# Zhijian-Mei/py-debruijn

Hardware: AMD Instinct MI355X
Metric: k-mers/s hashed+graph-built at k=31 (higher is better)
Workload: dtype u64; 1 GPU; 10000000 x 150 bp synthetic reads (10000000 per GPU): BASELINE.json configs[1]; k=31, 30x coverage of a 50000000 bp uniform genome, 1% substitutions, seed 1; k=31, reads_per_gpu=10000000, reads_total=10000000, read_len=150, parallelism=single table

## Files before the change

py-debruijn_amd/_dbg.py:

```python
from __future__ import annotations

import ctypes as C
import os

import numpy as np

_HERE = os.path.dirname(os.path.abspath(__file__))
LIB_PATH = os.environ.get("DBG_LIB") or os.path.join(_HERE, "libdbg_hip.so")

DBG_OK, DBG_E_ARG, DBG_E_HIP, DBG_E_ALPHABET, DBG_E_CAPACITY, DBG_E_NOMEM = 0, -1, -2, -3, -4, -5
F_INDEG, F_KEEP_MASK, F_KEEP_SHIFT, F_BRANCH, F_PULLED = 0x01, 0x1E, 1, 0x20, 0x40
NO_NODE = 0xFFFFFFFF
ABI_VERSION = 6

SYMBOLS = (
    "dbg_create", "dbg_destroy", "dbg_last_error", "dbg_abi_version", "dbg_set_option", "dbg_set_reads", "dbg_set_reads_fasta",
    "dbg_set_reads_fasta_file", "dbg_fasta_ingest_stats", "dbg_set_reads_fastq_file", "dbg_fastq_ingest_stats",
    "dbg_set_reads_fasta_records", "dbg_set_reads_fasta_records_file", "dbg_fasta_records_stats", "dbg_write_contigs_fasta_wrapped",
    "dbg_set_reads_device",
    "dbg_synth_reads", "dbg_reads_checksum", "dbg_copy_reads", "dbg_reads_device", "dbg_build", "dbg_refine_edge_order", "dbg_export_orders",
    "dbg_get_alphabet", "dbg_export_keepmask", "dbg_export_dict_order",
    "dbg_prune", "dbg_remove_tips",
    "dbg_mark_pull_reads", "dbg_walk", "dbg_get_sizes", "dbg_get_stats", "dbg_get_counter", "dbg_export_nodes", "dbg_export_keys_hi",
    "dbg_export_succ",
# ... 71 lines not shown
    _fields_ = [(n, C.c_uint64) for n in (
        "bytes_written", "chunks", "chunk_bytes", "peak_device_bytes", "lift_bytes")] + [
        (n, C.c_double) for n in ("ms_total", "ms_io_wait", "ms_fill", "ms_d2h")]

    def as_dict(self):
        return {n: getattr(self, n) for n, _ in self._fields_}


class SplitStats(C.Structure):
    _fields_ = [(n, C.c_uint64) for n in (
        "n_reads_in", "n_bytes_in", "n_reads_out", "n_bytes_out", "n_cut_bytes", "n_folded_bytes", "n_reads_changed",
        "n_reads_emptied", "changed", "peak_extra_device_bytes")]

    def as_dict(self):
        return {n: getattr(self, n) for n, _ in self._fields_}


SPLIT_FOLD_CASE = 1
SPLIT_WORD_BYTES = 64
SPLIT_BLOCK_BYTES = 256 * 4 * SPLIT_WORD_BYTES
SPLIT_ROUND_BYTES = 256 * SPLIT_BLOCK_BYTES


class RevcompStats(C.Structure):
    _fields_ = [(n, C.c_uint64) for n in (
        "n_reads_in", "n_bytes_in", "n_reads_out", "n_bytes_out", "n_other_bytes", "n_palindromes",
        "peak_extra_device_bytes")] + [("ms_kernel", C.c_double)]

    def as_dict(self):
        return {n: getattr(self, n) for n, _ in self._fields_}


RC_TILE_BYTES = 256 * 8 * 16
RC_SLICE_READS = 1024


class Spectrum(C.Structure):
    _fields_ = [(n, C.c_uint64) for n in ("n_nodes", "n_edges", "sum_edge_counts", "max_edge_count", "max_out_weight")] + [
        ("D", C.c_uint64 * 33), ("K", C.c_uint64 * 33)] + [
        (n, C.c_uint64) for n in ("pruned", "n_bins", "peak_extra_device_bytes")] + [("ms_kernel", C.c_double)]

    def as_dict(self):
        return {n: (np.array(getattr(self, n), dtype=np.uint64) if n in ("D", "K") else getattr(self, n)) for n, _ in self._fields_}


SP_LDS_BINS = 1024
SP_MAX_BINS = 1 << 20


class WalkBlock(C.Structure):
    _fields_ = [("src", C.c_void_p), ("contigs", C.c_void_p), ("n", C.c_uint64)]


COUNTERS = ("extract_presplit_fallbacks", "extract_presplit_rehists", "resolve_direct_hits", "resolve_keyed",
            "refine_crowded", "pull_crowded", "lookup_index_builds", "lookup_dir_calls", "lookup_index_calls",
            "part_lookup_calls", "count_events", "count_extra_ranges", "count_retries_query_cap", "count_retries_node_cap",
            "count_retries_counter16")


class DbgError(RuntimeError):
    def __init__(self, code, msg):
        super().__init__(f"dbg error {code}: {msg}")
        self.code = code


class AlphabetError(DbgError, ValueError):
    pass


_lib = None


def load_library():
    global _lib
    if _lib is not None:
        return _lib
    if not os.path.exists(LIB_PATH):
        raise OSError(f"{LIB_PATH} not found: build it with py-debruijn_amd/csrc/build.sh "
                      f"(there is no CPU fallback for the device path)")
    try:
        import torch
    except ImportError:
        pass
    lib = C.CDLL(LIB_PATH)
    H = C.c_void_p
    u64p, u32p, u8p = C.POINTER(C.c_uint64), C.POINTER(C.c_uint32), C.POINTER(C.c_uint8)
    vp = C.c_void_p
    sig = {
        "dbg_create": (C.c_int, [C.c_int, C.POINTER(H)]),
        "dbg_destroy": (None, [H]),
        "dbg_last_error": (C.c_char_p, [H]),
        "dbg_abi_version": (C.c_int, []),
        "dbg_set_option": (C.c_int, [H, C.c_char_p, C.c_int64]),
        "dbg_set_reads": (C.c_int, [H, vp, vp, C.c_uint64]),
        "dbg_set_reads_fasta": (C.c_int, [H, vp, C.c_uint64]),
        "dbg_set_reads_fasta_file": (C.c_int, [H, C.c_char_p, C.c_uint64, C.c_uint64, C.c_uint64]),
        "dbg_fasta_ingest_stats": (C.c_int, [H, C.POINTER(IngestStats)]),
        "dbg_set_reads_fastq_file": (C.c_int, [H, C.c_char_p, C.c_uint64, C.c_uint64, C.c_uint64, C.c_uint32]),
        "dbg_fastq_ingest_stats": (C.c_int, [H, C.POINTER(FastqStats)]),
        "dbg_set_reads_fasta_records": (C.c_int, [H, vp, C.c_uint64]),
        "dbg_set_reads_fasta_records_file": (C.c_int, [H, C.c_char_p, C.c_uint64, C.c_uint64, C.c_uint64]),
        "dbg_fasta_records_stats": (C.c_int, [H, C.POINTER(FastaRecordsStats)]),
        "dbg_set_reads_device": (C.c_int, [H, vp, C.c_uint64, vp, C.c_uint64]),
        "dbg_synth_reads": (C.c_int, [H, C.c_uint64, C.c_uint64, C.c_uint64, C.c_uint64, C.c_uint32, C.c_uint32]),
        "dbg_reads_checksum": (C.c_int, [H, u64p]),
        "dbg_copy_reads": (C.c_int, [H, vp, vp]),
        "dbg_build": (C.c_int, [H, C.c_int, C.c_uint64]),
# ... 965 lines not shown
```

py-debruijn_amd/csrc/dbg_hip.hip:

```cpp
#include <hip/hip_runtime.h>

#include <algorithm>
#include <chrono>
#include <cstdlib>
#include <cstdio>
#include <cstring>
#include <string>
#include <vector>

#include <cerrno>
#include <fcntl.h>
#include <sys/stat.h>
#include <unistd.h>

#include <rocprim/device/device_radix_sort.hpp>

#include "../../include/dbg.h"
#include "dbg_device.h"
#include "dbg_sk.h"
#include "dbg_sk2.h"
#include "dbg_sk3.h"
#include "dbg_wsk2.h"
#include "dbg_generic.h"
#include "dbg_genref.h"
// ... 1192 lines not shown
        h->n_edge_inst = sc[2];
        h->stats.ms_count = t_count.stop();
        h->stats.count_launches = 1;
        Timer t_c(h->stream);
        const uint64_t n_words = cap / 32;
        if ((rc = dev_alloc(h, &word_rank, n_words)) != DBG_OK) break;
        uint64_t n = 0;
        if ((rc = exclusive_scan(h, n_words, PopcWords{occ}, word_rank, &n)) != DBG_OK) break;
        h->n_nodes = n;
        if ((rc = dev_alloc(h, &h->d_keys, n)) != DBG_OK) break;
        if ((rc = dev_alloc(h, &h->d_stamps, n)) != DBG_OK) break;
        if ((rc = dev_alloc(h, &h->d_flags, n)) != DBG_OK) break;
        if ((rc = dev_alloc(h, &h->d_cnt, n * GEN_D)) != DBG_OK) break;
        if ((rc = dev_alloc(h, &h->d_succ, n * GEN_D)) != DBG_OK) break;
        if ((rc = dev_alloc(h, &h->d_deg, n)) != DBG_OK) break;
        if ((rc = dev_alloc(h, &h->d_keepmask, n)) != DBG_OK) break;
        if ((rc = dev_alloc(h, &h->d_rank_mc, n * GEN_D)) != DBG_OK) break;
        if ((rc = dev_alloc(h, &h->d_rank_fs, n * GEN_D)) != DBG_OK) break;
        if ((rc = dev_alloc(h, &estamp, n * GEN_D)) != DBG_OK) break;
        if (n) {
            (void)hipMemsetAsync(h->d_cnt, 0, n * GEN_D * 4, h->stream);
            (void)hipMemsetAsync(h->d_succ, 0xFF, n * GEN_D * 4, h->stream);
            (void)hipMemsetAsync(estamp, 0xFF, n * GEN_D * 8, h->stream);
            (void)hipMemsetAsync(h->d_keepmask, 0, n * 4, h->stream);
            hipLaunchKernelGGL(k_g_gather, dim3(grid_for(n_words, 256)), dim3(256), 0, h->stream, nodes, occ, word_rank, n_words,
                               h->d_keys, h->d_stamps, h->d_flags);
            hipLaunchKernelGGL(k_g_edges, dim3(grid_for(cap, 256)), dim3(256), 0, h->stream, edges, cap, nodes, cap - 1, k,
                               h->d_cnt, h->d_succ, estamp, (unsigned long long *)h->d_scalars);
            hipLaunchKernelGGL(k_g_rank, dim3(grid_for(n, 256)), dim3(256), 0, h->stream, n, h->d_cnt, estamp, h->d_rank_mc,
                               h->d_rank_fs, h->d_deg);
        }
        if (hipMemcpyAsync(sc, h->d_scalars, 8, hipMemcpyDeviceToHost, h->stream) != hipSuccess ||
            hipStreamSynchronize(h->stream) != hipSuccess) { h->err = "generic graph assembly failed"; rc = DBG_E_HIP; break; }
        if (sc[0] & STATUS_SUCC_MISSING) { h->err = "internal: edge endpoint missing from the node table"; rc = DBG_E_HIP; break; }
        h->stats.ms_succ = t_c.stop();
        h->order_exact = true;
    } while (0);
    cleanup();
    return rc;
}

extern "C" int dbg_set_option(dbg_t *h, const char *name, int64_t value) {
    if (!h || !name) return DBG_E_ARG;
    const std::string n(name);
    if (n == "engine" && (value == 0 || value == 1)) { h->engine = (int)value; return DBG_OK; }
    if (n == "bucket_bits" && value >= 0 && value <= SK_BUCKET_BITS) { h->bucket_bits = (int)value; return DBG_OK; }
    if (n == "lds_slots" && (value == 2048 || value == 4096)) { h->lds_slots = (int)value; return DBG_OK; }
    if (n == "phase_limit" && value >= 0 && value <= 5) { h->phase_limit = (int)value; return DBG_OK; }
    if (n == "estimate_scale_pct" && value >= 1 && value <= 1000) { h->est_scale_pct = (int)value; return DBG_OK; }
    if (n == "target_distinct" && value >= 0 && value <= 4096) { h->target_distinct = (int)value; return DBG_OK; }
    if (n == "shard_stamp64" && (value == 0 || value == 1)) { h->shard_stamp64 = (int)value; return DBG_OK; }
    if (n == "extract_generic" && (value == 0 || value == 1)) { h->extract_generic = (int)value; return DBG_OK; }
    if (n == "extract_presplit" && value >= 0 && value <= SK_PS_MAX_F0) { h->extract_presplit = (int)value; return DBG_OK; }
    if (n == "refine_streaming" && (value == 0 || value == 1)) { h->refine_streaming = value != 0; return DBG_OK; }
    if (n == "walk_jump_min_nodes" && value >= 0) { h->walk_jump_min = (uint64_t)value; return DBG_OK; }
    if (n == "wide_engine" && (value == 0 || value == 1)) { h->wide_engine = (int)value; return DBG_OK; }
    if (n == "count_kernel" && value >= 1 && value <= 3) { h->count_kernel = (int)value; return DBG_OK; }
    if (n == "stamp64" && (value == 0 || value == 1)) { h->stamp64 = (int)value; return DBG_OK; }
    if (n == "resolve_sorted" && value >= 0 && value <= 2) { h->resolve_sorted = (int)value; return DBG_OK; }
    if (n == "resolve_direct" && (value == 0 || value == 1)) { h->resolve_direct = (int)value; return DBG_OK; }
    if (n == "resolve_count" && (value == 0 || value == 1)) { h->resolve_count = (int)value; return DBG_OK; }
    if (n == "wcount_kernel" && (value == 1 || value == 2)) { h->wcount_kernel = (int)value; return DBG_OK; }
    if (n == "count_kernel_u64" && value >= 1 && value <= 3) { h->count_kernel_u64 = (int)value; return DBG_OK; }
    if (n == "lookup_index" && (value == 0 || value == 1)) { h->lookup_index = (int)value; return DBG_OK; }
    if (n == "ctgout_chunk_bytes" && value >= 0 && dbgk::co_chunk_ok((uint64_t)value)) { h->ctgout_chunk = (uint64_t)value; return DBG_OK; }
    if (n == "spectrum_variant" && value >= 0 && value <= 3) { h->spectrum_variant = (int)value; return DBG_OK; }
    if (n == "part_final_walk_steps" && value >= 1) { h->part_final_steps = (uint64_t)value; return DBG_OK; }
    if (n == "shard_node_limit" && value >= 0 && value < (1ll << 29)) { h->shard_node_limit = (uint64_t)value; return DBG_OK; }
    h->err = "unknown option or value out of range: " + n;
    return DBG_E_ARG;
}

static int build_wide_once(dbg *h, int k, uint64_t table_capacity_hint, bool packed, bool *overflow) {
    if (h->n_bytes >= (1ull << 43)) { h->err = "reads too large for the 44-bit positions of the table's protocol word"; return DBG_E_CAPACITY; }
    uint64_t want = table_capacity_hint;
    if (!want) {
        uint64_t inst = 0;
        CHK(reduce_sum(h, h->n_reads, KmerInstances{h->d_offsets, (uint64_t)k}, &inst));
        want = (uint64_t)((double)(inst + 1) / 0.7);
    }
    const uint64_t cap = std::max<uint64_t>(1024, (want + 1023) / 1024 * 1024);
    const uint64_t pk_words = (h->n_bytes + 31) / 32, n_occ = cap / 32;
    uint64_t *pk = nullptr;
    WSlot *tab = nullptr;
    uint32_t *tcnt = nullptr, *word_rank = nullptr;
    uint8_t *occ = nullptr;
    auto cleanup = [&]() {};
    int rc = DBG_OK;
    uint64_t sc[4] = {0, 0, 0, 0};
    do {
        Timer t(h->stream);
        if ((rc = buf_ensure(h, h->ar_wide[WIDE_PACKED], (pk_words + 3) * 8)) != DBG_OK) break;
        if ((rc = buf_ensure(h, h->ar_wide[WIDE_TABLE], cap * sizeof(WSlot))) != DBG_OK) break;
        if (!packed && (rc = buf_ensure(h, h->ar_wide[WIDE_TCNT], cap * 16)) != DBG_OK) break;
        if ((rc = buf_ensure(h, h->ar_wide[WIDE_OCC], cap)) != DBG_OK) break;
        if ((rc = buf_ensure(h, h->ar_wide[WIDE_WORD_RANK], n_occ * 4)) != DBG_OK) break;
        pk = (uint64_t *)h->ar_wide[WIDE_PACKED].p;
        tab = (WSlot *)h->ar_wide[WIDE_TABLE].p;
        tcnt = packed ? nullptr : (uint32_t *)h->ar_wide[WIDE_TCNT].p;
        occ = (uint8_t *)h->ar_wide[WIDE_OCC].p;
        word_rank = (uint32_t *)h->ar_wide[WIDE_WORD_RANK].p;
        (void)hipMemsetAsync(pk + pk_words, 0, 3 * 8, h->stream);
        hipLaunchKernelGGL(k_wtab_init, dim3(grid_for(cap, 256)), dim3(256), 0, h->stream, tab, cap);
        if (tcnt) (void)hipMemsetAsync(tcnt, 0, cap * 16, h->stream);
        (void)hipMemsetAsync(occ, 0, cap, h->stream);
        (void)hipMemsetAsync(h->d_scalars, 0, 64 * 8, h->stream);
// ... 812 lines not shown
        h->walk_indexed = true;
    } while (0);
    cleanup();
    h->stats.ms_walk = t.stop();
    return rc;
}

extern "C" int dbg_walk(dbg_t *h, int final_mode, uint64_t max_chars) {
    if (!h || !h->pruned) { if (h) h->err = "dbg_prune must run first"; return DBG_E_ARG; }
    HIPCHK(h, hipSetDevice(h->device));
    if (h->D == GEN_D) return walk_impl(h, gen_view(h), final_mode, max_chars);
    return walk_impl(h, dna_view(h), final_mode, max_chars);
}

extern "C" int dbg_get_sizes(dbg_t *h, dbg_sizes_t *o) {
    if (!h || !o) return DBG_E_ARG;
    if (h->k && h->n_nodes && !h->starts_known) {
        HIPCHK(h, hipSetDevice(h->device));
        CHK(ensure_starts(h));
    }
    memset(o, 0, sizeof(*o));
    o->k = h->k;
    o->abi_version = DBG_ABI_VERSION;
    o->n_reads = h->n_reads + h->nk_reads;
    o->n_bytes = h->n_bytes + h->nk_bytes;
    o->n_kmer_instances = h->n_kmer_inst;
    o->n_edge_instances = h->n_edge_inst;
    o->table_capacity = h->cap;
    o->n_nodes = h->n_nodes;
    o->n_edges = h->n_edges;
    o->n_branch = h->n_branch;
    o->n_pulled = h->n_pulled;
    o->n_pull_reads = h->n_pull_reads;
    o->n_starts = h->n_starts;
    o->n_contigs = h->n_contigs;
    o->contig_chars = h->contig_chars;
    o->tip_rounds = h->tip_rounds;
    o->contigs_materialised = h->walked ? 1 : 0;
    o->max_degree = (uint64_t)h->D;
    return DBG_OK;
}

extern "C" int dbg_get_stats(dbg_t *h, dbg_stats_t *o) {
    if (!h || !o) return DBG_E_ARG;
    *o = h->stats;
    return DBG_OK;
}

extern "C" int dbg_get_counter(dbg_t *h, const char *name, uint64_t *out) {
    if (!h || !name || !out) return DBG_E_ARG;
    const std::string n(name);
    if (n == "extract_presplit_rehists") { *out = h->presplit_rehists; return DBG_OK; }
    if (n == "extract_presplit_fallbacks") { *out = h->presplit_fallbacks; return DBG_OK; }
    if (n == "refine_crowded") { *out = h->refine_crowded; return DBG_OK; }
    if (n == "pull_crowded") { *out = h->pull_crowded; return DBG_OK; }
    if (n == "resolve_direct_hits") { *out = h->resolve_direct_hits; return DBG_OK; }
    if (n == "resolve_keyed") { *out = h->resolve_keyed; return DBG_OK; }
    if (n == "lookup_index_builds") { *out = h->lookup_index_builds; return DBG_OK; }
    if (n == "lookup_dir_calls") { *out = h->lookup_dir_calls; return DBG_OK; }
    if (n == "lookup_index_calls") { *out = h->lookup_index_calls; return DBG_OK; }
    if (n == "part_lookup_calls") { *out = h->part_lookup_calls; return DBG_OK; }
    if (n == "count_events") { *out = h->count_paths.events; return DBG_OK; }
    if (n == "count_extra_ranges") { *out = h->count_paths.extra_ranges; return DBG_OK; }
    if (n == "count_retries_query_cap") { *out = h->count_paths.retries_query_cap; return DBG_OK; }
    if (n == "count_retries_node_cap") { *out = h->count_paths.retries_node_cap; return DBG_OK; }
    if (n == "count_retries_counter16") { *out = h->count_paths.retries_counter16; return DBG_OK; }
    h->err = "unknown counter: " + n;
    return DBG_E_ARG;
}

#define D2H(h, dst, src, bytes)                                                                       do {                                                                                                  if ((dst) && (bytes)) HIPCHK(h, hipMemcpyAsync((dst), (src), (bytes), hipMemcpyDeviceToHost, (h)->stream));     } while (0)

extern "C" int dbg_export_nodes(dbg_t *h, uint64_t *keys, uint64_t *stamps, uint32_t *counts, uint8_t *flags) {
    if (!h || !h->k) return DBG_E_ARG;
    HIPCHK(h, hipSetDevice(h->device));
    CHK(ensure_dense(h));
    if (keys && !h->d_keys) memset(keys, 0, h->n_nodes * 8);
    else D2H(h, keys, h->d_keys, h->n_nodes * 8);
    D2H(h, stamps, h->d_stamps, h->n_nodes * 8);
    D2H(h, counts, h->d_cnt, h->n_nodes * 4 * h->D);
    D2H(h, flags, h->d_flags, h->n_nodes);
    HIPCHK(h, hipStreamSynchronize(h->stream));
    return DBG_OK;
}

extern "C" int dbg_export_keys_hi(dbg_t *h, uint64_t *keys_hi) {
    if (!h || !h->k || !keys_hi) return DBG_E_ARG;
    HIPCHK(h, hipSetDevice(h->device));
    if (!h->d_keys_hi) {
        memset(keys_hi, 0, h->n_nodes * 8);
        return DBG_OK;
    }
    D2H(h, keys_hi, h->d_keys_hi, h->n_nodes * 8);
    HIPCHK(h, hipStreamSynchronize(h->stream));
    return DBG_OK;
}

extern "C" int dbg_export_succ(dbg_t *h, uint32_t *succ) {
    if (!h || !h->k) return DBG_E_ARG;
    HIPCHK(h, hipSetDevice(h->device));
    CHK(ensure_dense(h));
    D2H(h, succ, h->d_succ, h->n_nodes * 4 * h->D);
    HIPCHK(h, hipStreamSynchronize(h->stream));
    return DBG_OK;
}

// ... 364 lines not shown
struct CeilDiv {
    const uint64_t *cnt;
    uint64_t d;
    __device__ uint64_t operator()(uint64_t i) const { return (cnt[i] + d - 1) / d; }
};

template <class ST, bool HAS_ST, class STI = ST, int STHI = 0>
static int multisplit_level(dbg *h, const uint64_t *p_start, const uint64_t *p_cnt, uint32_t n_seg, uint32_t spg,
                            uint64_t total, const uint64_t *in_w0, const uint64_t *in_w1, const STI *in_st,
                            uint64_t *out_w0, uint64_t *out_w1, ST *out_st, int shift, int nb, uint64_t *c_start,
                            uint64_t *c_cnt, dbg::Buf &b_scpre, dbg::Buf &b_cmat, dbg::Buf &b_offs, int fbits = 0,
                            const uint64_t *seg_add = nullptr, unsigned long long *d_sums = nullptr,
                            const uint64_t *host_cnt = nullptr, const uint32_t *ready_cmat = nullptr) {
    CHK(buf_ensure(h, b_scpre, (uint64_t)(n_seg + 1) * 8));
    uint64_t *sc_pre = (uint64_t *)b_scpre.p;
    uint64_t nsc = 0;
    if (ready_cmat) {
        std::vector<uint64_t> &pre = h->host_scpre;
        pre.resize((size_t)n_seg + 1);
        for (uint32_t i = 0; i <= n_seg; ++i) pre[i] = i;
        nsc = n_seg;
        HIPCHK(h, hipMemcpyAsync(sc_pre, pre.data(), pre.size() * 8, hipMemcpyHostToDevice, h->stream));
    } else if (host_cnt) {
        std::vector<uint64_t> &pre = h->host_scpre;
        pre.resize((size_t)n_seg + 1);
        for (uint32_t i = 0; i < n_seg; ++i) { pre[i] = nsc; nsc += (host_cnt[i] + MS_SC - 1) / MS_SC; }
        pre[n_seg] = nsc;
        HIPCHK(h, hipMemcpyAsync(sc_pre, pre.data(), pre.size() * 8, hipMemcpyHostToDevice, h->stream));
    } else {
        CHK(exclusive_scan(h, n_seg, CeilDiv{p_cnt, (uint64_t)MS_SC}, sc_pre, &nsc));
        HIPCHK(h, hipMemcpyAsync(sc_pre + n_seg, &nsc, 8, hipMemcpyHostToDevice, h->stream));
    }
    MsParents P{p_start, p_cnt, sc_pre, n_seg, spg};
    const uint64_t n_log = nsc * (uint64_t)nb;
    if (!ready_cmat) CHK(buf_ensure(h, b_cmat, n_log * 4));
    CHK(buf_ensure(h, b_offs, n_log * 8));
    const uint32_t *cmat = ready_cmat ? ready_cmat : (const uint32_t *)b_cmat.p;
    uint64_t *offs = (uint64_t *)b_offs.p;
    if (nsc) {
        if (ready_cmat)
            ;
        else if (d_sums)
            hipLaunchKernelGGL(HIP_KERNEL_NAME(k_ms_hist<true>), dim3((unsigned)nsc), dim3(256), 0, h->stream, P, in_w1, shift, nb,
                               fbits, (uint32_t *)b_cmat.p, d_sums);
        else
            hipLaunchKernelGGL(HIP_KERNEL_NAME(k_ms_hist<false>), dim3((unsigned)nsc), dim3(256), 0, h->stream, P, in_w1, shift, nb,
                               fbits, (uint32_t *)b_cmat.p, (unsigned long long *)nullptr);
        HIPCHK(h, hipGetLastError());
        CHK(exclusive_scan(h, n_log, MsLogical{P, cmat, nb}, offs, (uint64_t *)nullptr));
    }
    const uint64_t n_child = (uint64_t)(n_seg / spg) * nb;
    hipLaunchKernelGGL(k_ms_children, dim3(grid_for(n_child, 256)), dim3(256), 0, h->stream, P, offs, nb, total, c_start,
                       c_cnt);
    if (nsc) {
        auto kern = k_ms_scatter<ST, HAS_ST, STI, STHI>;
        const size_t lds = sizeof(MsLds<ST>);
        HIPCHK(h, hipFuncSetAttribute((const void *)kern, hipFuncAttributeMaxDynamicSharedMemorySize, (int)lds));
        hipLaunchKernelGGL(kern, dim3((unsigned)nsc), dim3(MS_NT), lds, h->stream, P, in_w0, in_w1, in_st, seg_add, shift, nb,
                           fbits, offs, out_w0, out_w1, out_st);
    }
    HIPCHK(h, hipGetLastError());
    return DBG_OK;
}

static void sk_provisional_bits(const dbg *h, uint64_t n_inst, double own, double target, int shard_bits, bool presplit_senders,
                                int l1_wide_from, int *T_out, int *l1_out) {
    constexpr int T_MAX = 20;
    int T = h->bucket_bits;
    if (T == 0) {
        const double want = (double)n_inst * own * 0.4 / target;
        while (T < T_MAX && (double)(1ull << T) < want) ++T;
    }
    if (T < shard_bits) T = shard_bits;
    if (presplit_senders) T = std::max(9, T);
    *T_out = T;
    *l1_out = T < 9 ? T : (T >= l1_wide_from && !presplit_senders ? 10 : 9);
}

template <int CAP> constexpr double SK_TARGET_DISTINCT = CAP * 0.36;

struct ExtractSplit {
    double target = 0.0;
    int f0 = 0;
    uint32_t n_wg = 0;
    int l1 = 0;
    const uint32_t *cmat = nullptr;
};

template <class ST>
static int sk_extract(dbg *h, int k, uint64_t *w0[2], uint64_t *w1[2], ST *st[2], uint64_t **seg_start_out,
                      uint64_t **seg_cnt_out, uint32_t *n_seg_out, uint64_t *n_rec_out, int part = 0, int n_parts = 1,
                      ExtractSplit *xs = nullptr) {
    const int m = sk_m_for_k(k), w = k - m + 1;
    unsigned long long *sc_dev = (unsigned long long *)h->d_scalars;
    const uint64_t all_tiles = (h->n_bytes + TILE - 1) / TILE;
    const uint64_t tile_first = all_tiles * (uint64_t)part / (uint64_t)n_parts;
    const uint64_t tiles = all_tiles * (uint64_t)(part + 1) / (uint64_t)n_parts - tile_first;
    uint64_t sc[8] = {0};
    uint32_t n_wg = (uint32_t)std::min<uint64_t>(std::max<uint64_t>(tiles, 1), 2048);
    uint64_t tiles_per_wg = (tiles + n_wg - 1) / n_wg;
    const double density = std::min(1.0, 2.6 / (double)(w + 1) + 1.3 * (double)(h->n_reads + 1) / (double)(h->n_bytes + 1) + 0.01);
    uint64_t seg_cap = (w == 1) ? tiles_per_wg * TILE : (uint64_t)((double)(tiles_per_wg * TILE) * density) + 256;
    int f0 = (xs && n_parts == 1 && tiles && m == SK_MAX_M && w <= 19 && !h->extract_generic) ? h->extract_presplit : 0;
    constexpr double PS_SLACK = 1.5;
    const uint32_t n_wg_plain = n_wg;
    const uint64_t seg_cap_plain = seg_cap;
    uint64_t n_seg = n_wg;
    int ps_l1 = 0;
    if (f0) {
        const uint64_t F0 = 1ull << f0;
        const double per_tile = (w == 1 ? 1.0 : density) * TILE * PS_SLACK / (double)F0;
        const uint64_t tpw_max = std::max<uint64_t>(1, (uint64_t)((double)(MS_SC - 64) / per_tile));
        int n_cu = 0;
        HIPCHK(h, hipDeviceGetAttribute(&n_cu, hipDeviceAttributeMultiprocessorCount, h->device));
        n_wg = (uint32_t)std::max<uint64_t>(std::min<uint64_t>(tiles, (uint64_t)n_cu * DBG_PS_WG_PER_CU), (tiles + tpw_max - 1) / tpw_max);
        tiles_per_wg = (tiles + n_wg - 1) / n_wg;
        seg_cap = std::min<uint64_t>(MS_SC, (uint64_t)((double)tiles_per_wg * per_tile) + 64);
        n_seg = (uint64_t)n_wg * F0;
        const uint64_t cut = h->n_reads * (uint64_t)(k - 1);
        int T_guess = 0;
        sk_provisional_bits(h, h->n_bytes > cut ? h->n_bytes - cut : 0, 1.0, xs->target, 0, false, DBG_L1_WIDE_FROM, &T_guess, &ps_l1);
        if (ps_l1 < f0) ps_l1 = 0;
    }
    std::vector<uint64_t> hseg;
    uint64_t *seg_start = nullptr, *seg_cnt = nullptr, *seg_nk = nullptr, *seg_ne = nullptr;
    uint32_t *ps_cmat = nullptr;
    uint64_t n_rec = 0;
    Timer t(h->stream);
    for (int attempt = 0; attempt < 3; ++attempt) {
        CHK(buf_ensure(h, h->ar_misc[MISC_SEGMENTS], (n_seg * 2 + (uint64_t)n_wg * 2) * 8));
        seg_start = (uint64_t *)h->ar_misc[MISC_SEGMENTS].p; seg_cnt = seg_start + n_seg; seg_nk = seg_cnt + n_seg; seg_ne = seg_nk + n_wg;
        hseg.assign((size_t)(n_seg * 2 + (uint64_t)n_wg * 2), 0);
        if (f0 && ps_l1) {
            CHK(buf_ensure(h, h->ar_misc[MISC_MS_CMAT], n_seg * 4 << (ps_l1 - f0)));
            ps_cmat = (uint32_t *)h->ar_misc[MISC_MS_CMAT].p;
        }
        const uint64_t rec_cap = seg_cap * n_seg;
        for (int set = 0; set < 2; ++set) {
            CHK(buf_ensure(h, h->ar_rec[set][REC_W0], rec_cap * 8));
            CHK(buf_ensure(h, h->ar_rec[set][REC_W1], rec_cap * 8));
            CHK(buf_ensure(h, h->ar_rec[set][REC_ST], rec_cap * sizeof(ST)));
            w0[set] = (uint64_t *)h->ar_rec[set][REC_W0].p;
            w1[set] = (uint64_t *)h->ar_rec[set][REC_W1].p;
            st[set] = (ST *)h->ar_rec[set][REC_ST].p;
        }
        for (uint64_t g = 0; g < n_seg; ++g) hseg[g] = g * seg_cap;
        HIPCHK(h, hipMemcpyAsync(seg_start, hseg.data(), (size_t)n_seg * 8, hipMemcpyHostToDevice, h->stream));
        HIPCHK(h, hipMemsetAsync(seg_cnt, 0, (size_t)(n_seg + (uint64_t)n_wg * 2) * 8, h->stream));
        HIPCHK(h, hipMemsetAsync(h->d_scalars, 0, 64 * 8, h->stream));
        if (tiles) {
            bool launched = false;
            if (m == SK_MAX_M && !h->extract_generic) {
#define DBG_EXW_CASE(W_) case W_: \
                if (f0) hipLaunchKernelGGL(HIP_KERNEL_NAME(k_sk_extract_w<ST, W_, true>), dim3(n_wg), dim3(256), 0, h->stream, \
                                           h->d_bases, h->n_bytes, h->d_startbits, tiles, w0[0], w1[0], st[0], seg_cap, seg_cnt, \
                                           seg_nk, seg_ne, sc_dev, tile_first, f0, ps_l1, ps_l1 ? ps_cmat : (uint32_t *)nullptr); \
                else hipLaunchKernelGGL(HIP_KERNEL_NAME(k_sk_extract_w<ST, W_, false>), dim3(n_wg), dim3(256), 0, h->stream, \
                                        h->d_bases, h->n_bytes, h->d_startbits, tiles, w0[0], w1[0], st[0], seg_cap, seg_cnt, \
                                        seg_nk, seg_ne, sc_dev, tile_first, 0, 0, (uint32_t *)nullptr); \
                launched = true; break;
                switch (w) {
                    DBG_EXW_CASE(1) DBG_EXW_CASE(2) DBG_EXW_CASE(3) DBG_EXW_CASE(4) DBG_EXW_CASE(5) DBG_EXW_CASE(6) DBG_EXW_CASE(7)
                    DBG_EXW_CASE(8) DBG_EXW_CASE(9) DBG_EXW_CASE(10) DBG_EXW_CASE(11) DBG_EXW_CASE(12) DBG_EXW_CASE(13)
                    DBG_EXW_CASE(14) DBG_EXW_CASE(15) DBG_EXW_CASE(16) DBG_EXW_CASE(17) DBG_EXW_CASE(18) DBG_EXW_CASE(19)
                    default: break;
                }
#undef DBG_EXW_CASE
            }
// ... 3572 lines not shown
```

py-debruijn_amd/csrc/dbg_hip_handle.h:

```cpp

enum MiscSlot {
    MISC_SEGMENTS,
    MISC_L1_CHILDREN,
    MISC_MS_SCPRE,
    MISC_MS_CMAT,
    MISC_MS_OFFS,
    MISC_BUCKETS,
    MISC_RANGES,
    MISC_QUERY_SEGS,
    MISC_ESTIMATE_SET,
    MISC_SLOTS
};


enum NodeSlot {
    NODE_KEYS,
    NODE_STAMPS64,
    NODE_CNT,
    NODE_FLAGS,
    NODE_ORDER,
    NODE_SUCC,
    NODE_DEG,
    NODE_STAMPS32,
    NODE_SLOTS
// ... 141 lines not shown
    bool starts_known = false;
    struct { const uint64_t *w0 = nullptr, *w1 = nullptr; const void *st = nullptr; int st_bytes = 0;
             const uint64_t *b_start = nullptr, *b_cnt = nullptr; bool valid = false; } sk_src;
    uint64_t *d_ctg_off = nullptr;
    char *d_ctg_chars = nullptr;
    uint64_t *d_ctg_score = nullptr, *d_ctg_stamp = nullptr;
    uint32_t *d_ctg_seq = nullptr;
    uint32_t *d_ctg_start = nullptr;
    uint32_t *d_lift = nullptr;
    int lift_levels = 0;
    bool walked = false;
    bool walk_final = false;
    bool walk_indexed = false;
    bool walk_sizes_only = false;
    uint64_t part_final_steps = dbgk::FW_DEFAULT_STEPS;
    uint64_t walk_jump_min = 1ull << 14;

    int D = 4, sym_bits = 2, n_sym = 0;
    bool alpha_known = false, is_dna = true;
    uint8_t alphabet[32] = {0};
    uint8_t *d_lut = nullptr;
    char *d_alpha = nullptr;
    uint32_t *d_keepmask = nullptr;
    uint8_t *d_rank_mc = nullptr, *d_rank_fs = nullptr;

    int engine = 0;
    int bucket_bits = 0;
    int lds_slots = 4096;
    int phase_limit = 0;
    int est_scale_pct = 100;
    int wide_engine = 1;
    int count_kernel_u64 = 3;
    int stamp64 = 0;
    int resolve_sorted = 0;
    int resolve_direct = 1;
    int resolve_count = 0;
    uint64_t resolve_direct_hits = 0, resolve_keyed = 0;
    int wcount_kernel = 2;
    int count_kernel = 2;

    struct Buf {
        void *p = nullptr;
        uint64_t bytes = 0;
    };
    Buf ar_rec[PINGPONG_SETS][REC_COLS], ar_q[PINGPONG_SETS][Q_COLS], ar_node[NODE_SLOTS], ar_misc[MISC_SLOTS], ar_csr[CSR_SLOTS], ar_dir, ar_l2, ar_scan, ar_shard[SHARD_SLOTS], ar_walk[WALK_SLOTS], ar_wide[WIDE_SLOTS], ar_refine[REFINE_SLOTS], ar_tips[TIPS_SLOTS], ar_part[SHARD_EXTRACT_PARTS][REC_COLS] ;
    int sk_T = 0, sk_l1 = 0, sk_l2 = 0, sk_nb2 = 0 , sk_cap = 0;
    bool refine_streaming = false;
    int target_distinct = 0;
    int shard_stamp64 = 0;
    int extract_generic = 0;
    int extract_presplit = DBG_EXTRACT_PRESPLIT;
    struct CountPaths { uint64_t events = 0, extra_ranges = 0, retries_query_cap = 0, retries_node_cap = 0, retries_counter16 = 0; } count_paths;
    uint64_t presplit_rehists = 0;
    uint64_t presplit_fallbacks = 0;
    uint64_t refine_crowded = 0, pull_crowded = 0;
    uint64_t sk_n_ranges = 0, sk_n_buckets = 0;
    SkGeom sk_geom{};
    void *shard_state = nullptr;
    void *multipass = nullptr;
    bool dropping_parts = false;
    dbg *spare_part = nullptr;
    bool wide_owner = false;
    bool borrowed_stream = false;
    bool arena_freed = false;
    std::vector<uint64_t> host_seg_cnt;
    std::vector<uint64_t> host_scpre;
    uint64_t shard_node_limit = 0;
    bool partial_graph = false;
    bool shard_open = false;
    int spectrum_variant = 3;
    uint64_t *d_btab = nullptr;
    uint64_t btab_cap = 0;
    struct NkBlock {
        uint64_t n_src = 0, n_reads = 0;
        uint32_t *next = nullptr, *z = nullptr, *start = nullptr;
    };
    bool nk_graph = false;
    uint64_t nk_reads = 0, nk_bytes = 0;
    std::vector<NkBlock> nk_blocks;
    uint8_t *d_nk_read_flags = nullptr;

    bool dir_valid = false;
    int lookup_index = 0;
    Buf ar_lookup[LOOKUP_SLOTS];
    bool lookup_built = false;
    uint64_t lookup_index_builds = 0, lookup_dir_calls = 0, lookup_index_calls = 0;
    bool part_dir_ok = false;
    uint64_t part_lookup_calls = 0;

    dbg_stats_t stats{};
    dbg_ingest_stats_t ingest{};
    dbg_fastq_stats_t fastq{};
    dbg_fasta_records_stats_t fasta_rec{};
    dbg_contig_out_stats_t ctgout{};
    uint64_t ctgout_chunk = 0;
};

struct ShardState {
    int n_shards = 0, my_shard = 0, shard_bits = 0, k = 0;
    std::vector<uint64_t> q_start, q_cnt;
    uint64_t n_remote = 0;
    uint64_t n_kmer_inst_local = 0;
    std::vector<uint64_t> l1_counts;
    int rec_words = 1, rec_stamp_bytes = 4;
};
static ShardState &shard_of(dbg *h);
// ... 97 lines not shown
```

py-debruijn_amd/csrc/dbg_sk.h:

```cpp
#pragma once
#include <cstddef>
#include "dbg_device.h"
#include "dbg_dir.h"
#include "dbg_minwin.h"

namespace dbgk {

constexpr int SK_MAX_M = 13;
constexpr int SK_BUCKET_BITS = 22;
constexpr int SK_META_BITS = 28;

__host__ __device__ inline int sk_m_for_k(int k) { return k < SK_MAX_M ? k : SK_MAX_M; }

__host__ __device__ inline uint32_t fmix32(uint32_t x) {
    x ^= x >> 16; x *= 0x85EBCA6Bu;
    x ^= x >> 13; x *= 0xC2B2AE35u;
    x ^= x >> 16;
    return x;
}
__device__ inline uint32_t bucket_hash22(uint32_t mmer) { return fmix32(mmer * 0x9E3779B1u + 0x7F4A7C15u) >> (32 - SK_BUCKET_BITS); }

__device__ inline uint32_t kmer_bucket22(uint64_t kmer, int k, int m) {
    const int w = k - m + 1;
    const uint32_t mmask = (uint32_t)((1ull << (2 * m)) - 1);
// ... 110 lines not shown
            int len;
            if (stop) {
                len = 1 + (__ffsll((unsigned long long)stop) - 1);
            } else {
                const unsigned long long stop2 = s.sbits[wd + 1] | ~s.vbits[wd + 1];
                len = 1 + room + (__ffsll((unsigned long long)stop2) - 1);
            }
            if (j + len > TILE) len = TILE - j;
            const uint64_t p = tile0 + j;
            const uint32_t s0 = startwin32(s.t, j) & 1u;
            const uint32_t sk_last = (startwin32(s.t, j + len - 1) >> k) & 1u;
            const uint32_t has_succ = sk_last ^ 1u;
            const int nb = k + len - 1 + (int)has_succ;
            uint64_t w0 = window32(s.t, j);
            uint64_t hi = window32(s.t, j + 32);
            if (nb < 32) { w0 &= ~0ull << (64 - 2 * nb); hi = 0; }
            else if (nb == 32) hi = 0;
            else hi &= ~0ull << (64 - 2 * (nb - 32));
            const uint32_t mp = j + s.minp[j];
            const uint32_t bh = bucket_hash22((uint32_t)(window32(s.t, mp) >> (64 - 2 * m)));
            const uint64_t w1 = (hi & (~0ull << SK_META_BITS)) | ((uint64_t)bh << 6) | ((uint64_t)(len - 1) << 1) | has_succ;
            const uint64_t o = gbase + r;
            rec_w0[o] = w0;
            rec_w1[o] = w1;
            rec_st[o] = (ST)((p << 1) | (s0 ^ 1u));
        }
    }
    if (overflow && threadIdx.x == 0) atomicOr(&scalars[0], STATUS_SEGMENT_FULL);
    n_k = wave_sum_u64(n_k);
    n_e = wave_sum_u64(n_e);
    __syncthreads();
    if ((threadIdx.x & 63) == 0) { red[threadIdx.x >> 6] = n_k; red[4 + (threadIdx.x >> 6)] = n_e; }
    __syncthreads();
    if (threadIdx.x == 0) {
        seg_cnt[blockIdx.x] = cursor;
        seg_nk[blockIdx.x] = red[0] + red[1] + red[2] + red[3];
        seg_ne[blockIdx.x] = red[4] + red[5] + red[6] + red[7];
    }
}

struct SkLdsW {
    TileLds t;
    uint8_t minp[TILE];
    unsigned long long sbits[TILE / 64 + 1];
    unsigned long long vbits[TILE / 64 + 1];
    uint32_t wpre[TILE / 64 + 1];
    uint16_t list[TILE];
    uint8_t edge[256];
    alignas(16) uint32_t nx[4][20];
    uint32_t nrec;
};

#ifndef DBG_EXW_WAVES
#define DBG_EXW_WAVES 3
#endif
constexpr int SK_PS_MAX_F0 = 6;
template <bool PS> struct SkLdsPs {};
template <> struct SkLdsPs<true> {
    uint32_t cur[1 << SK_PS_MAX_F0];
    uint32_t h1[1024];
    uint32_t ovf;
};
template <class ST, int W, bool PS = false>
__global__ __launch_bounds__(256, DBG_EXW_WAVES) void k_sk_extract_w(const char *__restrict__ bases, uint64_t n_bytes,
                                                      const uint32_t *__restrict__ startbits, uint64_t n_tiles,
                                                      uint64_t *rec_w0, uint64_t *rec_w1, ST *rec_st, uint64_t seg_cap,
                                                      uint64_t *seg_cnt, uint64_t *seg_nk, uint64_t *seg_ne,
                                                      unsigned long long *scalars , uint64_t tile_first,
                                                      int f0 = 0, int l1 = 0, uint32_t *cmat = nullptr) {
    constexpr int M = SK_MAX_M, K = W + M - 1, NV = 32 + W - 1;
    static_assert(TILE == 256 * 32, "one lane per 32 positions");
    static_assert(K <= 31 && NV + M - 1 <= 64, "window must fit the two 32-base registers");
    __shared__ SkLdsW s;
    __shared__ SkLdsPs<PS> ps;
    __shared__ uint64_t red[8];
    if constexpr (PS) {
        for (int i = threadIdx.x; i < 1024; i += 256) ps.h1[i] = 0;
        if (threadIdx.x < (1 << SK_PS_MAX_F0)) ps.cur[threadIdx.x] = 0;
        if (threadIdx.x == 0) ps.ovf = 0;
    }
    const uint64_t t_beg = tile_first + n_tiles * blockIdx.x / gridDim.x, t_end = tile_first + n_tiles * (blockIdx.x + 1) / gridDim.x;
    const uint64_t seg0 = (uint64_t)blockIdx.x * seg_cap;
    uint64_t cursor = 0;
    uint64_t n_k = 0, n_e = 0;
    bool overflow = false;
    const int j0 = threadIdx.x * 32;
    for (uint64_t tile = t_beg; tile < t_end; ++tile) {
        const uint64_t tile0 = tile * TILE;
        __syncthreads();
        if constexpr (PS) {
            if (ps.ovf) { overflow = true; break; }
        }
        const uint32_t bad = load_tile(s.t, bases, n_bytes, startbits, tile0);
        if (bad) atomicOr(&scalars[0], STATUS_BAD_BASE);
        __syncthreads();
        const uint64_t wa = window32(s.t, j0), wb = window32(s.t, j0 + 32);
        uint32_t pv[NV];
#pragma unroll
        for (int i = 0; i < 32; ++i) {
            const uint64_t win = (i == 0) ? wa : ((wa << (2 * i)) | (wb >> (64 - 2 * i)));
            pv[i] = mmer_packed((uint32_t)(win >> (64 - 2 * M)), (uint32_t)i);
        }
        const int lane = threadIdx.x & 63, wave = threadIdx.x >> 6;
        if constexpr (W > 1) {
            if (lane < W - 1)
                s.nx[wave][lane] = mmer_packed((uint32_t)(window32(s.t, (wave + 1) * 2048 + lane) >> (64 - 2 * M)), 32u + (uint32_t)lane);
            __builtin_amdgcn_fence(__ATOMIC_RELEASE, "wavefront");
// ... 82 lines not shown
            if (nb < 32) { w0 &= ~0ull << (64 - 2 * nb); hi = 0; }
            else if (nb == 32) hi = 0;
            else hi &= ~0ull << (64 - 2 * (nb - 32));
            const uint32_t mp = (j & ~31) + s.minp[(j & ~31) + index_byte_at(j & 31)];
            const uint32_t bh = bucket_hash22((uint32_t)(window32(s.t, mp) >> (64 - 2 * M)));
            const uint64_t w1 = (hi & (~0ull << SK_META_BITS)) | ((uint64_t)bh << 6) | ((uint64_t)(len - 1) << 1) | has_succ;
            uint64_t o = gbase + r;
            if constexpr (PS) {
                const uint32_t c = bh >> (SK_BUCKET_BITS - f0);
                const uint32_t rk = atomicAdd(&ps.cur[c], 1u);
                if (cmat) atomicAdd(&ps.h1[bh >> (SK_BUCKET_BITS - l1)], 1u);
                if (rk >= seg_cap) { ps.ovf = 1; continue; }
                o = ((uint64_t)c * gridDim.x + blockIdx.x) * seg_cap + rk;
            }
            rec_w0[o] = w0;
            rec_w1[o] = w1;
            rec_st[o] = (ST)((p << 1) | (s0 ^ 1u));
        }
    }
    n_k = wave_sum_u64(n_k);
    n_e = wave_sum_u64(n_e);
    __syncthreads();
    if constexpr (PS) {
        if (ps.ovf) overflow = true;
        if (threadIdx.x < (1 << f0))
            seg_cnt[(uint64_t)threadIdx.x * gridDim.x + blockIdx.x] = min(ps.cur[threadIdx.x], (uint32_t)seg_cap);
        if (cmat) {
            const int nbg = 1 << (l1 - f0);
            for (int d = threadIdx.x; d < (1 << l1); d += 256)
                cmat[((uint64_t)(d >> (l1 - f0)) * gridDim.x + blockIdx.x) * nbg + (d & (nbg - 1))] = ps.h1[d];
        }
    }
    if (overflow && threadIdx.x == 0) atomicOr(&scalars[0], STATUS_SEGMENT_FULL);
    if ((threadIdx.x & 63) == 0) { red[threadIdx.x >> 6] = n_k; red[4 + (threadIdx.x >> 6)] = n_e; }
    __syncthreads();
    if (threadIdx.x == 0) {
        if constexpr (!PS) seg_cnt[blockIdx.x] = cursor;
        seg_nk[blockIdx.x] = red[0] + red[1] + red[2] + red[3];
        seg_ne[blockIdx.x] = red[4] + red[5] + red[6] + red[7];
    }
}

#ifndef DBG_MS_CH
#define DBG_MS_CH 4096
#endif
constexpr int MS_CH = DBG_MS_CH;
template <class ST> struct MsChunk { static constexpr int CH = sizeof(ST) == 8 ? MS_CH : MS_CH + MS_CH / 2; };
constexpr int MS_SC = 32768;
constexpr int MS_MAX_NB = 1024;
#ifndef DBG_MS_NT
#define DBG_MS_NT 512
#endif
constexpr int MS_NT = DBG_MS_NT;

struct MsParents {
    const uint64_t *start;
    const uint64_t *cnt;
    const uint64_t *sc_pre;
    uint32_t n_seg;
    uint32_t spg;
};

__device__ inline void ms_locate(const MsParents &P, uint64_t g, uint32_t *seg, uint64_t *sidx) {
    uint32_t lo = 0, hi = P.n_seg;
    while (hi - lo > 1) {
        const uint32_t mid = (lo + hi) >> 1;
        if (P.sc_pre[mid] <= g) lo = mid; else hi = mid;
    }
    *seg = lo;
    *sidx = g - P.sc_pre[lo];
}

__device__ inline uint32_t ms_child(uint64_t w1, int shift, int nb, int fbits) {
    const uint32_t v = (uint32_t)(w1 >> shift);
    return fbits ? (uint32_t)(((uint64_t)(v & ((1u << fbits) - 1u)) * (uint32_t)nb) >> fbits) : (v & (uint32_t)(nb - 1));
}

template <bool SUMS>
__global__ __launch_bounds__(256) void k_ms_hist(MsParents P, const uint64_t *__restrict__ w1, int shift, int nb, int fbits,
                                                 uint32_t *cmat, unsigned long long *sums) {
    __shared__ uint32_t hist[MS_MAX_NB];
    uint32_t seg;
    uint64_t sidx;
    ms_locate(P, blockIdx.x, &seg, &sidx);
    for (int b = threadIdx.x; b < nb; b += 256) hist[b] = 0;
    __syncthreads();
    const uint64_t beg = P.start[seg] + sidx * MS_SC;
    const uint64_t end = min(P.start[seg] + P.cnt[seg], beg + (uint64_t)MS_SC);
    uint64_t n_inst = 0, n_edge = 0;
    for (uint64_t i = beg + threadIdx.x; i < end; i += 256) {
        const uint64_t x = w1[i];
        atomicAdd(&hist[ms_child(x, shift, nb, fbits)], 1u);
        if (SUMS) { n_inst += ((x >> 1) & 31) + 1; n_edge += ((x >> 1) & 31) + (x & 1); }
    }
    __syncthreads();
    for (int b = threadIdx.x; b < nb; b += 256) cmat[(uint64_t)blockIdx.x * nb + b] = hist[b];
    if (SUMS) {
        n_inst = wave_sum_u64(n_inst);
        n_edge = wave_sum_u64(n_edge);
        if ((threadIdx.x & 63) == 0) {
            if (n_inst) atomicAdd(&sums[0], (unsigned long long)n_inst);
            if (n_edge) atomicAdd(&sums[1], (unsigned long long)n_edge);
        }
    }
}

// ... 99 lines not shown
                }
                rk[i] = atomicAdd(&s.hist[ms_child(r1[i], shift, nb, fbits)], 1u);
            }
        }
        __syncthreads();
        MS_TICK(2);
        {
            constexpr int EPT = MS_MAX_NB / MS_NT;
            const int b0 = threadIdx.x * EPT;
            uint32_t h4[EPT];
            uint64_t sum = 0;
#pragma unroll
            for (int j = 0; j < EPT; ++j) { h4[j] = (b0 + j < nb) ? s.hist[b0 + j] : 0; sum += h4[j]; }
            uint64_t tot;
            uint32_t ex = (uint32_t)block_exscan<MS_NT / 64>(sum, &tot);
#pragma unroll
            for (int j = 0; j < EPT; ++j) { if (b0 + j < nb) s.start[b0 + j] = ex; ex += h4[j]; }
        }
        __syncthreads();
        MS_TICK(3);
#pragma unroll
        for (int i = 0; i < CH / MS_NT; ++i) {
            const int q = i * MS_NT + threadIdx.x;
            if (q < n) {
                const uint32_t b = ms_child(r1[i], shift, nb, fbits);
                const uint32_t d = s.start[b] + rk[i];
                s.w0[d] = r0[i];
                s.w1[d] = r1[i];
                if (HAS_ST) s.st[d] = rs[i];
            }
        }
        __syncthreads();
        MS_TICK(4);
        for (int q = threadIdx.x; q < n; q += MS_NT) {
            const uint64_t x1 = s.w1[q];
            const uint32_t b = ms_child(x1, shift, nb, fbits);
            const uint64_t g = s.run[b] + (q - s.start[b]);
            out_w0[g] = s.w0[q];
            out_w1[g] = x1;
            if (HAS_ST) out_st[g] = s.st[q];
        }
        __syncthreads();
        MS_TICK(5);
        for (int b = threadIdx.x; b < nb; b += MS_NT) s.run[b] += s.hist[b];
        __syncthreads();
        MS_TICK(6);
    }
#ifdef DBG_MS_PROF
    if (threadIdx.x == 0) {
        for (int i = 0; i < 7; ++i) atomicAdd(&g_ms_prof[i], prof_[i]);
        atomicAdd(&g_ms_prof[7], 1ull);
    }
#endif
}


template <class ST>
__global__ __launch_bounds__(256) void k_estimate_distinct(const uint64_t *__restrict__ b_start,
                                                           const uint64_t *__restrict__ b_cnt, uint32_t bucket,
                                                           const uint64_t *__restrict__ rec_w0,
                                                           const uint64_t *__restrict__ rec_w1, int k,
                                                           unsigned long long *set, uint64_t set_mask,
                                                           unsigned long long *out ) {
    const uint64_t beg = b_start[bucket], n = b_cnt[bucket];
    uint64_t inst = 0, fresh = 0;
    for (uint64_t r = (uint64_t)blockIdx.x * blockDim.x + threadIdx.x; r < n; r += (uint64_t)gridDim.x * blockDim.x) {
        const uint64_t w0 = rec_w0[beg + r], w1 = rec_w1[beg + r];
        const uint64_t hi = w1 & (~0ull << SK_META_BITS);
        const int len = (int)((w1 >> 1) & 31) + 1;
        for (int i = 0; i < len; ++i) {
            const uint64_t kmer = (i ? (w0 << (2 * i)) | (hi >> (64 - 2 * i)) : w0) >> (64 - 2 * k);
            ++inst;
            uint64_t slot = mix64(kmer) & set_mask;
            for (uint64_t probe = 0; probe <= set_mask; ++probe) {
                unsigned long long cur = set[slot];
                if (cur == EMPTY_KEY) {
                    cur = atomicCAS(&set[slot], EMPTY_KEY, (unsigned long long)kmer);
                    if (cur == EMPTY_KEY) { ++fresh; break; }
                }
                if (cur == kmer) break;
                slot = (slot + 1) & set_mask;
            }
        }
    }
    inst = wave_sum_u64(inst);
    fresh = wave_sum_u64(fresh);
    if ((threadIdx.x & 63) == 0) {
        if (inst) atomicAdd(&out[0], (unsigned long long)inst);
        if (fresh) atomicAdd(&out[1], (unsigned long long)fresh);
    }
}

struct SkRange {
    uint32_t bucket;
    uint32_t mask, val;
    uint32_t node_cnt;
    uint64_t node_base;
    uint32_t next;
    uint32_t pad;
};

__device__ inline uint32_t fold32(uint64_t kmer) { return (uint32_t)kmer * 0x9E3779B1u ^ (uint32_t)(kmer >> 32) * 0x85EBCA77u; }
__device__ inline uint32_t sub_hash(uint64_t kmer) { return fmix32(fold32(kmer) ^ 0x27D4EB2Fu); }
__device__ inline uint32_t slot_hash(uint64_t kmer) {
    const uint32_t lo = (uint32_t)kmer, hi = (uint32_t)(kmer >> 32);
    return (lo ^ (hi << 11) ^ (hi >> 7) ^ (lo >> 15)) * 0x9E3779B1u;
// ... 673 lines not shown
```

Baseline: 58.52 billion k-mers/s.

## Add small-fanout multisplit scatter kernel and tunable extract grid

```diff
diff --git a/py-debruijn_amd/_dbg.py b/py-debruijn_amd/_dbg.py
--- a/py-debruijn_amd/_dbg.py
+++ b/py-debruijn_amd/_dbg.py
@@ -147,7 +147,8 @@
     _fields_ = [("src", C.c_void_p), ("contigs", C.c_void_p), ("n", C.c_uint64)]
 
 
-COUNTERS = ("extract_presplit_fallbacks", "extract_presplit_rehists", "resolve_direct_hits", "resolve_keyed",
+COUNTERS = ("extract_presplit_fallbacks", "extract_presplit_rehists", "ms_scatter_small", "ms_scatter_wide",
+            "resolve_direct_hits", "resolve_keyed",
             "refine_crowded", "pull_crowded", "lookup_index_builds", "lookup_dir_calls", "lookup_index_calls",
             "part_lookup_calls", "count_events", "count_extra_ranges", "count_retries_query_cap", "count_retries_node_cap",
             "count_retries_counter16")
diff --git a/py-debruijn_amd/csrc/dbg_hip.hip b/py-debruijn_amd/csrc/dbg_hip.hip
--- a/py-debruijn_amd/csrc/dbg_hip.hip
+++ b/py-debruijn_amd/csrc/dbg_hip.hip
@@ -1268,6 +1268,7 @@
     if (n == "shard_stamp64" && (value == 0 || value == 1)) { h->shard_stamp64 = (int)value; return DBG_OK; }
     if (n == "extract_generic" && (value == 0 || value == 1)) { h->extract_generic = (int)value; return DBG_OK; }
     if (n == "extract_presplit" && value >= 0 && value <= SK_PS_MAX_F0) { h->extract_presplit = (int)value; return DBG_OK; }
+    if (n == "extract_grid" && value >= 0 && value <= 65535) { h->extract_grid = (int)value; return DBG_OK; }
     if (n == "refine_streaming" && (value == 0 || value == 1)) { h->refine_streaming = value != 0; return DBG_OK; }
     if (n == "walk_jump_min_nodes" && value >= 0) { h->walk_jump_min = (uint64_t)value; return DBG_OK; }
     if (n == "wide_engine" && (value == 0 || value == 1)) { h->wide_engine = (int)value; return DBG_OK; }
@@ -2186,6 +2187,8 @@
     const std::string n(name);
     if (n == "extract_presplit_rehists") { *out = h->presplit_rehists; return DBG_OK; }
     if (n == "extract_presplit_fallbacks") { *out = h->presplit_fallbacks; return DBG_OK; }
+    if (n == "ms_scatter_small") { *out = h->ms_scatter_small; return DBG_OK; }
+    if (n == "ms_scatter_wide") { *out = h->ms_scatter_wide; return DBG_OK; }
     if (n == "refine_crowded") { *out = h->refine_crowded; return DBG_OK; }
     if (n == "pull_crowded") { *out = h->pull_crowded; return DBG_OK; }
     if (n == "resolve_direct_hits") { *out = h->resolve_direct_hits; return DBG_OK; }
@@ -2656,12 +2659,21 @@
     const uint64_t n_child = (uint64_t)(n_seg / spg) * nb;
     hipLaunchKernelGGL(k_ms_children, dim3(grid_for(n_child, 256)), dim3(256), 0, h->stream, P, offs, nb, total, c_start,
                        c_cnt);
-    if (nsc) {
+    constexpr bool HAS_SMALL = std::is_same<ST, STI>::value && STHI == 0;
+    bool small = false;
+    if constexpr (HAS_SMALL) small = nb <= MS_S_NB;
+    if (nsc && small) {
+        if constexpr (HAS_SMALL)
+            hipLaunchKernelGGL(HIP_KERNEL_NAME(k_ms_scatter_s<ST, HAS_ST>), dim3((unsigned)nsc), dim3(MS_NT), 0, h->stream, P, in_w0,
+                               in_w1, in_st, seg_add, shift, nb, fbits, offs, out_w0, out_w1, out_st);
+        ++h->ms_scatter_small;
+    } else if (nsc) {
         auto kern = k_ms_scatter<ST, HAS_ST, STI, STHI>;
         const size_t lds = sizeof(MsLds<ST>);
         HIPCHK(h, hipFuncSetAttribute((const void *)kern, hipFuncAttributeMaxDynamicSharedMemorySize, (int)lds));
         hipLaunchKernelGGL(kern, dim3((unsigned)nsc), dim3(MS_NT), lds, h->stream, P, in_w0, in_w1, in_st, seg_add, shift, nb,
                            fbits, offs, out_w0, out_w1, out_st);
+        ++h->ms_scatter_wide;
     }
     HIPCHK(h, hipGetLastError());
     return DBG_OK;
@@ -2717,7 +2729,9 @@
         const uint64_t tpw_max = std::max<uint64_t>(1, (uint64_t)((double)(MS_SC - 64) / per_tile));
         int n_cu = 0;
         HIPCHK(h, hipDeviceGetAttribute(&n_cu, hipDeviceAttributeMultiprocessorCount, h->device));
-        n_wg = (uint32_t)std::max<uint64_t>(std::min<uint64_t>(tiles, (uint64_t)n_cu * DBG_PS_WG_PER_CU), (tiles + tpw_max - 1) / tpw_max);
+        const uint64_t want_wg = h->extract_grid ? (uint64_t)h->extract_grid : (uint64_t)n_cu * DBG_PS_WG_PER_CU;
+        n_wg = (uint32_t)std::max<uint64_t>(std::min<uint64_t>(tiles, want_wg), (tiles + tpw_max - 1) / tpw_max);
+        if (n_wg > want_wg) n_wg = (uint32_t)std::min<uint64_t>(tiles, (n_wg + want_wg - 1) / want_wg * want_wg);
         tiles_per_wg = (tiles + n_wg - 1) / n_wg;
         seg_cap = std::min<uint64_t>(MS_SC, (uint64_t)((double)tiles_per_wg * per_tile) + 64);
         n_seg = (uint64_t)n_wg * F0;
diff --git a/py-debruijn_amd/csrc/dbg_hip_handle.h b/py-debruijn_amd/csrc/dbg_hip_handle.h
--- a/py-debruijn_amd/csrc/dbg_hip_handle.h
+++ b/py-debruijn_amd/csrc/dbg_hip_handle.h
@@ -217,6 +217,8 @@
     int extract_presplit = DBG_EXTRACT_PRESPLIT;
     struct CountPaths { uint64_t events = 0, extra_ranges = 0, retries_query_cap = 0, retries_node_cap = 0, retries_counter16 = 0; } count_paths;
     uint64_t presplit_rehists = 0;
+    int extract_grid = 0;
+    uint64_t ms_scatter_small = 0, ms_scatter_wide = 0;
     uint64_t presplit_fallbacks = 0;
     uint64_t refine_crowded = 0, pull_crowded = 0;
     uint64_t sk_n_ranges = 0, sk_n_buckets = 0;
diff --git a/py-debruijn_amd/csrc/dbg_sk.h b/py-debruijn_amd/csrc/dbg_sk.h
--- a/py-debruijn_amd/csrc/dbg_sk.h
+++ b/py-debruijn_amd/csrc/dbg_sk.h
@@ -186,7 +186,7 @@
 };
 
 #ifndef DBG_EXW_WAVES
-#define DBG_EXW_WAVES 3
+#define DBG_EXW_WAVES 4
 #endif
 constexpr int SK_PS_MAX_F0 = 6;
 template <bool PS> struct SkLdsPs {};
@@ -375,6 +375,10 @@
 #define DBG_MS_NT 512
 #endif
 constexpr int MS_NT = DBG_MS_NT;
+constexpr int MS_S_NB = 64;
+constexpr int MS_S_CH = 2048;
+constexpr int MS_S_WG_PER_CU = 3;
+static_assert(MS_S_NB <= 64 && MS_SC % MS_S_CH == 0, "small fan-out: one lane per child, whole rounds per super-chunk");
 
 struct MsParents {
     const uint64_t *start;
@@ -580,6 +584,92 @@
         atomicAdd(&g_ms_prof[7], 1ull);
     }
 #endif
+}
+
+template <class ST>
+struct MsLdsS {
+    uint64_t w0[MS_S_CH];
+    uint64_t w1[MS_S_CH];
+    ST st[MS_S_CH];
+    uint32_t hist[64];
+};
+
+template <class ST, bool HAS_ST>
+__global__ __launch_bounds__(MS_NT, MS_S_WG_PER_CU * MS_NT / 256) void k_ms_scatter_s(
+    MsParents P, const uint64_t *__restrict__ in_w0, const uint64_t *__restrict__ in_w1, const ST *__restrict__ in_st,
+    const uint64_t *__restrict__ seg_add, int shift, int nb, int fbits, const uint64_t *__restrict__ offs, uint64_t *out_w0,
+    uint64_t *out_w1, ST *out_st) {
+    __shared__ MsLdsS<ST> s;
+    constexpr int CH = MS_S_CH, R = CH / MS_NT;
+    constexpr uint64_t SC = MS_SC;
+    static_assert(CH % MS_NT == 0 && MS_S_WG_PER_CU * sizeof(MsLdsS<ST>) <= 160 * 1024, "small-fan-out chunk");
+    uint32_t seg;
+    uint64_t sidx;
+    ms_locate(P, blockIdx.x, &seg, &sidx);
+    const ST st_add = (HAS_ST && seg_add) ? (ST)seg_add[seg] : (ST)0;
+    const uint32_t grp = seg / P.spg;
+    const uint64_t g_lo = P.sc_pre[grp * P.spg], g_hi = P.sc_pre[(grp + 1) * P.spg];
+    const uint64_t nsc = g_hi - g_lo, gidx = (uint64_t)blockIdx.x - g_lo;
+    const int lane = threadIdx.x & 63;
+    const uint64_t run = lane < nb ? offs[(uint64_t)nb * g_lo + (uint64_t)lane * nsc + gidx] : 0;
+    uint32_t prev = 0;
+    if (threadIdx.x < 64) s.hist[threadIdx.x] = 0;
+    __syncthreads();
+    const uint64_t beg = P.start[seg] + sidx * SC;
+    const uint64_t end = min(P.start[seg] + P.cnt[seg], beg + SC);
+    for (uint64_t c0 = beg; c0 < end; c0 += CH) {
+        const int n = (int)min((uint64_t)CH, end - c0);
+        uint64_t r0[R], r1[R];
+        ST rs[R];
+        uint32_t rk[R];
+#pragma unroll
+        for (int i = 0; i < R; ++i) {
+            const int q = i * MS_NT + threadIdx.x;
+            r1[i] = 0;
+            if (q < n) {
+                r0[i] = in_w0[c0 + q];
+                r1[i] = in_w1[c0 + q];
+                if (HAS_ST) rs[i] = in_st[c0 + q] + st_add;
+                rk[i] = atomicAdd(&s.hist[ms_child(r1[i], shift, nb, fbits)], 1u);
+            }
+        }
+        __syncthreads();
+        const uint32_t cum = s.hist[lane];
+        const uint32_t cnt = cum - prev;
+        uint32_t inc = cnt;
+#pragma unroll
+        for (int d = 1; d < 64; d <<= 1) {
+            const uint32_t o = __shfl_up(inc, d, 64);
+            if (lane >= d) inc += o;
+        }
+        const uint32_t ex = inc - cnt;
+        const uint32_t slot0 = ex - prev;
+#pragma unroll
+        for (int i = 0; i < R; ++i) {
+            const int q = i * MS_NT + threadIdx.x;
+            const uint32_t b = ms_child(r1[i], shift, nb, fbits);
+            const uint32_t d0 = __shfl(slot0, (int)b, 64);
+            if (q < n) {
+                const uint32_t d = d0 + rk[i];
+                s.w0[d] = r0[i];
+                s.w1[d] = r1[i];
+                if (HAS_ST) s.st[d] = rs[i];
+            }
+        }
+        __syncthreads();
+        const unsigned long long gb = run + prev - ex;
+        for (int q0 = 0; q0 < n; q0 += MS_NT) {
+            const int q = q0 + threadIdx.x;
+            const uint64_t x1 = q < n ? s.w1[q] : 0;
+            const uint64_t g = __shfl(gb, (int)ms_child(x1, shift, nb, fbits), 64) + (uint64_t)q;
+            if (q < n) {
+                out_w0[g] = s.w0[q];
+                out_w1[g] = x1;
+                if (HAS_ST) out_st[g] = s.st[q];
+            }
+        }
+        prev = cum;
+    }
 }
 
 
```

Measured after the change: 59.41 billion k-mers/s, median of 6. 1.02x the previous value.
